# ZhangYizhao/UltraRE

Measured on AMD Instinct MI355X. Metric: training interactions/sec + unlearn retrain wall-time, ml-1m 5-shard SISA, higher is better.
Workload: dtype f32; 1 GPU; ml1m-shaped synthetic 6040x3416, 896914 train rows, 5-shard SISA (uniform grouping), d=32, batch=30000, SGD-momentum-L2, all shards of a rank side by side; parallelism=shards x1, arch=gfx950:sramecc+:xnack-

## Files before the change

include/ultrare_hip.h:

```cpp
#ifndef ULTRARE_HIP_H
#define ULTRARE_HIP_H

#include <stdint.h>

#ifdef __cplusplus
extern "C" {
#endif

#define URE_ABI_VERSION 15
#define URE_MAX_MODELS_PER_CALL 32
#define URE_SCORE_PARTIALS 2048

int ure_abi_version(void);
const char *ure_source_hash(void);
const char *ure_last_error(void);
int ure_device_info(int dev, int *n_cu, int *wave_size, char *arch, int arch_len);

typedef struct ure_shard {
    const int32_t *ent_oid;
    const float   *ent_r;
    uint16_t      *ent_tag;
    const int32_t *ent_src;
    uint16_t      *file_tag;
    uint32_t      *inv_stage;
// ... 32 lines not shown
typedef struct ure_job ure_job_t;

int ure_job_create(const ure_shard_t *shards, int n_shards, ure_job_t **out);

int ure_copy_rows_batch(int32_t n, const float *const *src, float *const *dst, float *const *dst2, const int64_t *rows, int32_t k, int32_t d,
                        void *stream);

int ure_epoch_sse_batch(int32_t n, const float *const *sse, const int64_t *n_user, int32_t epochs, double *out, void *stream);
int ure_job_destroy(ure_job_t *job);
int64_t ure_job_shard_steps(const ure_job_t *job, int s);
int64_t ure_job_ticks(const ure_job_t *job);

int ure_job_train(ure_job_t *job, int64_t tick0, int64_t tick1, void *stream);
int ure_job_materialize(ure_job_t *job, int64_t ticks_done, void *stream);
int ure_job_touch_rows(ure_job_t *job, int64_t *pairs, int64_t *window_steps);
int ure_job_index_read(ure_job_t *job, int shard, int which, void *out, int64_t capacity, int64_t *bytes);
int ure_job_train_profiled(ure_job_t *job, int64_t tick0, int64_t tick1, void *stream, double *step_ms,
                           int64_t *n_step, double *assign_ms, int64_t *n_assign);

int ure_host_randperm(const int64_t *seeds, int n_perms, int64_t n, int32_t *out, int n_threads);
int ure_host_randperm_tags(const int64_t *seeds, int n_perms, int64_t n, int32_t batch, uint16_t *tags, int n_threads);
typedef struct ure_perm {
    int64_t   seed;
    uint16_t *tags;
    int32_t   n;
    int32_t   batch;
} ure_perm_t;
int64_t ure_device_randperm_tags_scratch(int64_t n_max, int32_t groups);
int ure_device_randperm_tags(const ure_perm_t *perms, int32_t n_perms, int64_t n_max, uint32_t *scratch, int64_t scratch_words, int32_t groups,
                             void *stream);
// ... 147 lines not shown
```

ultrare_amd/_native.py:

```python
import ctypes
import os

import numpy as np

_PKG = os.path.dirname(os.path.abspath(__file__))
LIB_PATH = os.path.join(_PKG, 'libultrare_hip.so')
ABI_VERSION = 15
MAX_MODELS_PER_CALL = 32

_vp = ctypes.c_void_p
_i32 = ctypes.c_int32
_i64 = ctypes.c_int64


class UreShard(ctypes.Structure):
    _fields_ = [
        ('ent_oid', _vp), ('ent_r', _vp), ('ent_tag', _vp), ('ent_src', _vp), ('file_tag', _vp), ('inv_stage', _vp), ('inv_off', _vp),
        ('sched', _vp), ('units', _vp), ('n_units', _i32), ('n_active', _i32), ('n_slots', _i64),
        ('U', _vp * 2), ('V', _vp * 2), ('mU', _vp), ('mV', _vp),
        ('U0', _vp), ('V0', _vp), ('lr_host', _vp), ('lazy_rows', _i32),
        ('snapU', _vp), ('snapV', _vp), ('snap_a', _vp), ('snap', _vp), ('row_slot', _vp),
        ('perm', _vp), ('lr', _vp), ('sse', _vp),
        ('N', _i32), ('n_user', _i32), ('n_item', _i32), ('d', _i32),
        ('batch', _i32), ('epochs', _i32),
# ... 10 lines not shown
_PROTOTYPES = {
    'ure_abi_version': (ctypes.c_int, []),
    'ure_source_hash': (ctypes.c_char_p, []),
    'ure_last_error': (ctypes.c_char_p, []),
    'ure_device_info': (ctypes.c_int, [ctypes.c_int, ctypes.POINTER(ctypes.c_int), ctypes.POINTER(ctypes.c_int),
                                       ctypes.c_char_p, ctypes.c_int]),
    'ure_job_create': (ctypes.c_int, [ctypes.POINTER(UreShard), ctypes.c_int, ctypes.POINTER(_vp)]),
    'ure_job_destroy': (ctypes.c_int, [_vp]),
    'ure_copy_rows_batch': (ctypes.c_int, [_i32, _vp, _vp, _vp, _vp, _i32, _i32, _vp]),
    'ure_epoch_sse_batch': (ctypes.c_int, [_i32, _vp, _vp, _i32, _vp, _vp]),
    'ure_job_shard_steps': (_i64, [_vp, ctypes.c_int]),
    'ure_job_ticks': (_i64, [_vp]),
    'ure_job_train': (ctypes.c_int, [_vp, _i64, _i64, _vp]),
    'ure_job_materialize': (ctypes.c_int, [_vp, _i64, _vp]),
    'ure_job_touch_rows': (ctypes.c_int, [_vp, _vp, _vp]),
    'ure_job_index_read': (ctypes.c_int, [_vp, ctypes.c_int, ctypes.c_int, _vp, _i64, ctypes.POINTER(_i64)]),
    'ure_job_train_profiled': (ctypes.c_int, [_vp, _i64, _i64, _vp, ctypes.POINTER(ctypes.c_double), ctypes.POINTER(_i64),
                                              ctypes.POINTER(ctypes.c_double), ctypes.POINTER(_i64)]),
    'ure_host_randperm': (ctypes.c_int, [_vp, ctypes.c_int, _i64, _vp, ctypes.c_int]),
    'ure_host_randperm_tags': (ctypes.c_int, [_vp, ctypes.c_int, _i64, _i32, _vp, ctypes.c_int]),
    'ure_device_randperm_tags_scratch': (_i64, [_i64, _i32]),
    'ure_device_randperm_tags': (ctypes.c_int, [_vp, _i32, _i64, _vp, _i64, _i32, _vp]),
    'ure_device_shuffle_tags_scratch': (_i64, [_i64, _i32]),
    'ure_device_shuffle_tags_flag': (_i64, [_i64, _i32]),
    'ure_device_shuffle_tags': (ctypes.c_int, [_vp, _i32, _i64, _vp, _i64, _i32, _vp]),
    'ure_host_mt_advance': (ctypes.c_int, [_vp, _i64, _i64]),
    'ure_host_mt_jump_blocks': (ctypes.c_int, [_vp, _i64]),
    'ure_host_mt_jump_support': (ctypes.c_int, [_i64, _vp, _i32, ctypes.POINTER(_i32)]),
    'ure_host_mt_charpoly': (ctypes.c_int, [_vp, _i32]),
    'ure_host_draw_int64': (ctypes.c_int, [_vp, _i64, _i64, _i64, _vp]),
# ... 319 lines not shown
```

ultrare_amd/build.py:

```python
import os
import shutil
import subprocess
import sys

PKG = os.path.dirname(os.path.abspath(__file__))
ROOT = os.path.dirname(PKG)
CSRC = os.path.join(PKG, 'csrc')
LIB = os.path.join(PKG, 'libultrare_hip.so')
SOURCES = ['ure_common.hip', 'block_cache.cpp', 'mf_train.hip', 'tag_prep.hip', 'mf_eval.hip', 'mf_combine.hip', 'mf_ridge.hip', 'mf_recommend.hip', 'mf_rank.hip', 'pair_dist.hip', 'job_io.hip', 'perm_tags.hip', 'perm_chain.hip', 'mf_init.hip', 'ot.hip', 'ot_sinkhorn.hip', 'csr_group.hip', 'ot_solver.cpp', 'host_rng.cpp', 'mt_jump.cpp', 'host_layout.cpp']
FLAGS = ['-O3', '--offload-arch=gfx950', '-std=c++17', '-fPIC', '-shared', '-munsafe-fp-atomics',
         '-ffp-contract=off', '-Wall', '-Wno-unused-result', '-pthread', '-mllvm', '-amdgpu-kernarg-preload-count=8']


AVX2_SOURCE = 'host_normal_avx2.cpp'
AVX2_FLAGS = ['-O3', '-std=c++17', '-fPIC', '-mavx2', '-mfma', '-ffp-contract=fast', '-c']


def torch_include():
    try:
        import importlib.util
        spec = importlib.util.find_spec('torch')
        inc = os.path.join(os.path.dirname(spec.origin), 'include')
        return inc if os.path.exists(os.path.join(inc, 'ATen', 'native', 'cpu', 'avx_mathfun.h')) else None
    except Exception:
        return None


def source_hash(extra=()):
    import hashlib
    h = hashlib.sha256()
    files = sorted(os.path.join(CSRC, f) for f in os.listdir(CSRC) if not f.startswith('.')) + [os.path.join(ROOT, 'include', 'ultrare_hip.h')]
    for path in files:
        h.update(os.path.basename(path).encode() + b'\0')
        with open(path, 'rb') as f:
            h.update(f.read())
    h.update(' '.join(list(FLAGS) + list(extra) + AVX2_FLAGS + [str(torch_include() is not None)]).encode())
    return h.hexdigest()[:16]


STEP_KERNEL_FILES = ['mf_train.hip', 'mf_job.h', 'mf_touch.h', 'mf_index.h', 'tag_prep.h', 'tag_prep.hip', 'ure_internal.h']


def step_kernel_hash():
    import hashlib
    h = hashlib.sha256()
    for path in [os.path.join(CSRC, f) for f in STEP_KERNEL_FILES]:
        h.update(os.path.basename(path).encode() + b'\0')
        with open(path, 'rb') as f:
            h.update(f.read())
    with open(os.path.join(ROOT, 'include', 'ultrare_hip.h')) as f:
        text = f.read()
    a, b = text.index('typedef struct ure_shard'), text.index('} ure_shard_t;')
    h.update(text[a:b].encode())
    h.update(' '.join(FLAGS).encode())
    return h.hexdigest()[:16]
# ... 47 lines not shown
```

ultrare_amd/csrc/mf_job.h:

```cpp
#pragma once
#include <memory>

namespace ure {


static int check_descriptor(const ure_shard_t *shards, int k)
{
    const ure_shard_t &S = shards[k];
    const int n_rows = S.n_user + S.n_item;
    const bool ok = S.N > 0 && S.n_user > 0 && S.n_item > 0 && S.batch > 0 && S.epochs > 0 && pow2(S.d) && S.d >= 4 &&
                    S.d <= 256 && S.n_active >= 0 && S.n_active <= n_rows && S.units && S.n_units >= 0 &&
                    S.n_units % (kBlock / lanes_per_row(S.d)) == 0 && S.n_slots >= S.N && S.ent_oid && S.ent_r && S.ent_tag && S.ent_src &&
                    S.file_tag && S.sched && S.U[0] && S.U[1] && S.V[0] && S.V[1] && S.mU && S.mV && (S.perm || S.file_tags) && S.lr && S.sse &&
                    (!S.lazy_rows || (S.U0 && S.V0 && S.lr_host));
    if (!ok) return fail(-1, "ure_job_create: shard %d has an invalid descriptor", k);
    if (S.d != shards[0].d) return fail(-1, "ure_job_create: all shards of a job share d");
    const int steps = make_shard_aux(S).steps;
    if (steps > 65534) return fail(-1, "ure_job_create: shard %d needs %lld steps/epoch (> 65534)", k, (long long)steps);
    if (S.touch_mode && (S.n_multi < 0 || S.n_multi > S.n_active)) return fail(-1, "ure_job_create: shard %d: n_multi outside [0, n_active]", k);
    if (tag_partitioned(S.N) && !(S.inv_stage && S.inv_off)) return fail(-1, "ure_job_create: shard %d lacks inv_stage / inv_off", k);
    return 0;
}

static bool snapshot_set_ok(const ure_shard_t &S)
// ... 29 lines not shown
    }
    for (int k = 0; k < n_shards; ++k)
        if (!snapshot_set_ok(shards[k])) return fail(-1, "ure_job_create: shard %d has an incomplete snapshot set (full: snapU + snapV; compact: snap with lazy_rows; snap_a with lazy_rows)", k);
    for (int k = 0; k < n_shards && touch; ++k)
        if (const char *why = touch_refusal(shards, k, make_shard_aux(shards[k]).steps)) return fail(-1, "ure_job_create: touch mode refused for shard %d: %s", k, why);
    return 0;
}


static void plan_job(ure_job *job, const ure_shard_t *shards, int n_shards)
{
    job->host.assign(shards, shards + n_shards);
    job->d = shards[0].d;
    if (const char *e = std::getenv("URE_SHARD_FAST")) { job->shard_fast = e[0] != '0'; job->shard_sliced = e[0] == '2'; }
    if (const char *e = std::getenv("URE_INDEX_STAGED")) job->scatter_staged = e[0] != '0';
    job->ahead = shards[0].touch_mode == 2;
    job->index = shards[0].touch_mode == 3;
    for (int k = 0; k < n_shards; ++k) {
        const ure_shard_t &S = shards[k];
        const shard_aux A = make_shard_aux(S);
        const int n_rows = S.n_user + S.n_item, per_block = kBlock / lanes_per_row(S.d);
        job->aux_host.push_back(A);
        job->lr_host.emplace_back(S.lr_host ? std::vector<float>(S.lr_host, S.lr_host + S.epochs) : std::vector<float>());
        job->host[k].lr_host = nullptr;
        job->ticks = std::max(job->ticks, (int64_t)A.steps * S.epochs);
        job->row_blocks.push_back(S.touch_mode ? S.n_units / per_block + (S.n_active - S.n_multi + kBlock - 1) / kBlock
                                               : S.n_units / per_block + (S.lazy_rows ? 0 : (n_rows - S.n_active + per_block - 1) / per_block));
        job->max_n = std::max(job->max_n, S.N);
        job->max_slots = std::max(job->max_slots, S.n_slots);
        const bool small = tag_partitioned(S.N);
// ... 132 lines not shown
    int tab_n = kTouchTab;
    if (job->index)
        for (const shard_aux &A : job->aux_host) tab_n = std::max(tab_n, A.steps + 1);
    for (shard_aux &A : job->aux_host) A.ptab_stride = tab_n;
    const std::vector<float> tab = closed_form_table(job, tab_n);
    float4 *ptab = nullptr;
    if (hipError_t e = job_block(job, tab.size() * sizeof(float), kNoFill, &ptab)) return e;
    if (hipError_t e = hipMemcpy(ptab, tab.data(), tab.size() * sizeof(float), hipMemcpyHostToDevice)) return e;
    bool index_short = true;
    for (const shard_aux &A : job->aux_host) index_short = index_short && A.steps <= kIdxWin;
    for (int k = 0; k < (int)job->host.size(); ++k)
        if (hipError_t e = job->index ? index_memory(job, k, ptab, index_short) : window_memory(job, k, ptab)) return e;
    return hipSuccess;
}

static hipError_t upload_job(ure_job *job)
{
    const size_t n = job->host.size();
    if (hipError_t e = hipMalloc(&job->dev, sizeof(ure_shard_t) * n)) return e;
    if (hipError_t e = hipMemcpy(job->dev, job->host.data(), sizeof(ure_shard_t) * n, hipMemcpyHostToDevice)) return e;
    if (hipError_t e = hipMalloc(&job->dev_ab, sizeof(double) * 2 * n)) return e;
    if (job->touch)
        if (hipError_t e = touch_memory(job)) return e;
    if (hipError_t e = hipMalloc(&job->dev_aux, sizeof(shard_aux) * n)) return e;
    return hipMemcpy(job->dev_aux, job->aux_host.data(), sizeof(shard_aux) * n, hipMemcpyHostToDevice);
}

}

extern "C" int ure_job_create(const ure_shard_t *shards, int n_shards, ure_job_t **out)
{
    URE_ARG(shards && out && n_shards > 0 && n_shards <= 65535);
    if (int rc = ure::check_shards(shards, n_shards)) return rc;
    auto *job = new ure::ure_job();
    std::unique_ptr<ure_job_t, decltype(&ure_job_destroy)> hold(reinterpret_cast<ure_job_t *>(job), ure_job_destroy);
    ure::plan_job(job, shards, n_shards);
    const hipError_t e = ure::upload_job(job);
    if (e != hipSuccess) return ure::fail((int)e, "ure_job_create: %s", hipGetErrorString(e));
// ... 16 lines not shown
```

ultrare_amd/csrc/mf_train.hip:

```cpp
#include "tag_prep.h"

#include <algorithm>
#include <cstdlib>
#include <type_traits>
#include <vector>

#ifndef URE_KGB_NARROW
#define URE_KGB_NARROW 5
#endif
#ifndef URE_KGB_D16
#define URE_KGB_D16 5
#endif
#ifndef URE_WAVES_D16
#define URE_WAVES_D16 5
#endif
#ifndef URE_KGB_D8
#define URE_KGB_D8 5
#endif
#ifndef URE_WAVES_D8
#define URE_WAVES_D8 5
#endif
#ifndef URE_KGB_WIDE
#define URE_KGB_WIDE 4
#endif
// ... 35 lines not shown

template <int LPR, int V4>
__device__ __forceinline__ void mf_step(const ure_shard_t *__restrict__ shards, const shard_aux *__restrict__ aux, int64_t tick, int shard_fast)
{
    constexpr int D = LPR * V4 * 4;
    using Row = RowVec<V4>;
    constexpr int G = kWave / LPR;
    constexpr int UPB = kBlock / LPR;
    constexpr int CAP = kSegPerLane * LPR;
    constexpr int kGB = step_kgb(LPR, V4);
    constexpr int kQueueBytes = kWavesPerBlock * kQueue * 8;
    static_assert(kTagLds <= kQueueBytes, "tag phases must fit in the queue space");
    __shared__ __attribute__((aligned(16))) char lds_raw[kQueueBytes];
    __shared__ float4 part_acc[UPB][V4][LPR];
    int (*q_oid)[kQueue] = reinterpret_cast<int (*)[kQueue]>(lds_raw);
    float (*q_r)[kQueue] = reinterpret_cast<float (*)[kQueue]>(lds_raw + kWavesPerBlock * kQueue * 4);

    int shard_idx = (int)(shard_fast ? blockIdx.x : blockIdx.y);
    int wg = (int)(shard_fast ? blockIdx.y : blockIdx.x);
    if (shard_fast >> 1) {
        const unsigned n_sh = (unsigned)shard_fast >> 8;
        const unsigned x = blockIdx.x & 7u, j = blockIdx.x >> 3;
        const unsigned jq = j / n_sh, jr = j - jq * n_sh;
        const unsigned slice = n_sh * x + jr;
        shard_idx = (int)(slice >> 3);
        wg = (int)(jq * 8 + (slice & 7u));
    }
    const ure_shard_t &S = shards[shard_idx];
    const shard_aux &A = aux[shard_idx];
    {
        const int p_epochs = S.epochs, p_nu = S.n_user, p_ni = S.n_item, p_units = S.n_units, p_act = S.n_active, p_lazy = S.lazy_rows;
        const int64_t p_slots = S.n_slots;
        const float p_lam = S.lam, p_mu = S.mu;
        asm volatile("" ::"s"(p_epochs), "s"(p_nu), "s"(p_ni), "s"(p_units), "s"(p_act), "s"(p_lazy), "s"(p_slots), "s"(p_lam), "s"(p_mu),
                     "s"(S.lr), "s"(S.sched), "s"(S.units), "s"(S.ent_oid), "s"(S.ent_r), "s"(S.ent_tag), "s"(S.U[0]), "s"(S.U[1]),
                     "s"(S.V[0]), "s"(S.V[1]), "s"(S.mU), "s"(S.mV), "s"(S.sse), "s"(A.steps), "s"(A.inv_steps), "s"(A.ride_m),
                     "s"(A.ride_ab), "s"(A.ride_c), "s"(A.ranges), "s"(A.derive_blocks));
    }
    const int steps = A.steps;
    if (tick >= (int64_t)steps * S.epochs) return;
    const int epoch = (int)epoch_of(A, tick);
    const int s = (int)(tick - (int64_t)epoch * steps);
    const int cur = (int)(tick & 1);
    const bool first = tick == 0;
    const int n_rows = S.n_user + S.n_item;
    const int wave = threadIdx.x >> 6, lane = threadIdx.x & 63;
    const int sub = lane & (LPR - 1), grp = lane / LPR;
    const float lam = S.lam, mu = S.mu, lr = ldg(S.lr + epoch);
    const int32_t *__restrict__ ent_oid = S.ent_oid;
    const float *__restrict__ ent_r = S.ent_r;
    const uint16_t *__restrict__ ent_tag = S.ent_tag + (size_t)(epoch & 1) * S.n_slots;
    int *qo = q_oid[wave];
    float *qr = q_r[wave];

    auto sgd_update = [&](const Row &wr, const Row &mr, const Row &ar, float *mom_row, float *next_row, float *snap_row) {
        Row gr, nr;
#pragma unroll
        for (int i = 0; i < V4; ++i) {
            const float4 w = wr.q[i], m4 = mr.q[i], acc = ar.q[i];
            float4 g, wn;
            g.x = fmaf(lam, w.x, acc.x); g.y = fmaf(lam, w.y, acc.y);
            g.z = fmaf(lam, w.z, acc.z); g.w = fmaf(lam, w.w, acc.w);
            if (!first) {
                g.x = __fadd_rn(__fmul_rn(mu, m4.x), g.x); g.y = __fadd_rn(__fmul_rn(mu, m4.y), g.y);
                g.z = __fadd_rn(__fmul_rn(mu, m4.z), g.z); g.w = __fadd_rn(__fmul_rn(mu, m4.w), g.w);
            }
            wn.x = fmaf(-lr, g.x, w.x); wn.y = fmaf(-lr, g.y, w.y);
            wn.z = fmaf(-lr, g.z, w.z); wn.w = fmaf(-lr, g.w, w.w);
// ... 10 lines not shown
    const TagRide ride = tag_ride(A, s, epoch + 1 < S.epochs);
    const int nbR = ride.count;
    const int nbRows = nbU + nbD;
    const int blk = wg;
    if (blk >= nbRows) {
        const int rb = blk - nbRows;
        if (rb >= nbR) return;
        if (ride.phase == 0) tag_partition(S, epoch + 1, ride.first + rb, lds_raw);
        else if (ride.phase == 1) tag_collect(S, ride.first + rb, lds_raw);
        else tag_derive(S, epoch + 1, ride.first + rb, A.derive_blocks);
        return;
    }
    const int local = wave * G + grp;
    const bool dense_only = blk >= nbU;
    int4 du = make_int4(-1, 0, 0, local | (1 << 16));
    if (dense_only) {
        const int idx = S.n_active + (blk - nbU) * UPB + local;
        if (idx < n_rows) du.x = ldg(S.sched + 4 * (size_t)idx);
    } else {
        du = ldg_i4(S.units + 4 * ((size_t)blk * UPB + local));
    }
    const bool have = du.x >= 0;
    const int leader = du.w & 0xFFFF, count = (du.w >> 16) & 0x3FFF;
    const bool multi = (du.w >> 30) & 1;
    const bool owner = have && local == leader;
    const bool is_user = du.x < S.n_user;
    const int row = is_user ? du.x : du.x - S.n_user;
    const size_t row_off = (size_t)(have ? row : 0) * D;
    Row w = row_zero<V4>(), m4 = w, acc = w;
    if (have) {
        w = row_load<LPR, V4>((is_user ? S.U[cur] : S.V[cur]) + row_off, sub);
    }
    if (owner && !first) m4 = row_load<LPR, V4>((is_user ? S.mU : S.mV) + row_off, sub);
    const bool snap_here = S.snap != nullptr && S.row_slot != nullptr && s == steps - 1;
    int snap_slot = -1;
    if (snap_here && owner) snap_slot = ldg(S.row_slot + du.x);
    float sse = 0.f;
    URE_STAMP(2);
    if (!dense_only) {
        const float *__restrict__ other = is_user ? S.V[cur] : S.U[cur];
        int *gq = qo + grp * CAP;
        float *gr = qr + grp * CAP;
        const int beg = du.y, end = have ? du.z : 0;
        for (int seg = beg;; seg += CAP) {
            if (!__any(seg < end)) break;
            const int p0 = seg + sub * kSegPerLane;
            const bool valid = p0 < end;
            uint4 t4 = make_uint4(0xFFFFFFFFu, 0xFFFFFFFFu, 0xFFFFFFFFu, 0xFFFFFFFFu);
            int4 o0 = make_int4(0, 0, 0, 0), o1 = o0;
            float4 r0 = make_float4(0.f, 0.f, 0.f, 0.f), r1 = r0;
            if (valid) {
                t4 = ldg_u4(ent_tag + p0);
                o0 = ldg_i4(ent_oid + p0);
                o1 = ldg_i4(ent_oid + p0 + 4);
                r0 = ldg_f4(ent_r + p0);
                r1 = ldg_f4(ent_r + p0 + 4);
            }
            const unsigned tw[4] = {t4.x, t4.y, t4.z, t4.w};
            const int ov[8] = {o0.x, o0.y, o0.z, o0.w, o1.x, o1.y, o1.z, o1.w};
            const float rv[8] = {r0.x, r0.y, r0.z, r0.w, r1.x, r1.y, r1.z, r1.w};
            unsigned mb = 0;
#pragma unroll
            for (int k = 0; k < 8; ++k) {
                const unsigned tg = (tw[k >> 1] >> ((k & 1) * 16)) & 0xFFFFu;
                mb |= (tg == (unsigned)s ? 1u : 0u) << k;
            }
            const int c = __popc(mb);
            const int inc = group_scan<LPR>(c, sub);
            const int qn = (int)group_sum<LPR>((float)c);
            int mpos = inc - c, upos = qn + sub * kSegPerLane - mpos;
#pragma unroll
            for (int k = 0; k < 8; ++k) {
                const bool hit = (mb >> k) & 1u;
                const int pos = ((hit ? mpos : upos) + grp) & (CAP - 1);
                gq[pos] = ov[k];
                gr[pos] = rv[k];
                mpos += hit ? 1 : 0;
                upos += hit ? 0 : 1;
            }
            __builtin_amdgcn_wave_barrier();
            if (seg == beg) URE_STAMP(3);
            for (int t0 = 0; __any(t0 < qn); t0 += kGB) {
                int o[kGB];
                float r[kGB];
                bool act[kGB];
                Row v[kGB];
#pragma unroll
                for (int k = 0; k < kGB; ++k) {
                    const int qi = (min(t0 + k, CAP - 1) + grp) & (CAP - 1);
                    act[k] = t0 + k < qn;
                    o[k] = gq[qi];
                    r[k] = gr[qi];
                }
#pragma unroll
                for (int k = 0; k < kGB; ++k) v[k] = row_load<LPR, V4>(other + (size_t)(act[k] ? o[k] : 0) * D, sub);
#pragma unroll
                for (int k = 0; k < kGB; ++k) {
                    const float p = group_sum<LPR>(row_dot<V4>(w, v[k]));
                    const float e = p - r[k];
                    const float ge = act[k] ? 2.0f * e : 0.0f;
                    if (act[k]) sse = fmaf(e, e, sse);
                    row_axpy<V4>(acc, ge, v[k]);
                }
            }
            __builtin_amdgcn_wave_barrier();
        }
        URE_STAMP(4);
        if (multi) {
            if (have && count > 1) {
#pragma unroll
                for (int i = 0; i < V4; ++i) part_acc[local][i][sub] = acc.q[i];
                if (sub == 0) qr[grp * CAP] = sse;
            }
            __syncthreads();
            if (owner && count > 1) {
#pragma unroll
                for (int i = 0; i < V4; ++i) {
                    float4 a4 = part_acc[leader][i][sub];
                    for (int k = 1; k < count; ++k) {
                        const float4 t = part_acc[leader + k][i][sub];
                        a4.x += t.x; a4.y += t.y; a4.z += t.z; a4.w += t.w;
                    }
                    acc.q[i] = a4;
                }
                sse = 0.f;
                for (int k = 0; k < count; ++k) sse += q_r[(leader + k) / G][((leader + k) % G) * CAP];
            }
        }
    }
    if (owner) {
        sgd_update(w, m4, acc, (is_user ? S.mU : S.mV) + row_off, (is_user ? S.U[cur ^ 1] : S.V[cur ^ 1]) + row_off,
                   snap_slot >= 0 ? S.snap + ((size_t)epoch * S.n_active + snap_slot) * D : nullptr);
        if (is_user && sub == 0 && sse != 0.f) {
            float *slot = S.sse + (size_t)epoch * S.n_user + row;
            stg(slot, ldg(slot) + sse);
        }
    }
}

template <int LPR, int V4>
__global__ __launch_bounds__(kBlock) __attribute__((amdgpu_waves_per_eu(step_waves(LPR, V4)))) void mf_step_kernel(const ure_shard_t *__restrict__ shards, const shard_aux *__restrict__ aux, int64_t tick, int shard_fast)
// ... 353 lines not shown
    auto mark = [&](std::vector<hipEvent_t> *v) -> int {
        if (!v) return 0;
        hipEvent_t e;
        URE_HIP(hipEventCreate(&e));
        v->push_back(e);
        URE_HIP(hipEventRecord(e, st));
        return 0;
    };
    auto timed = [&](std::vector<hipEvent_t> *v, auto launches) -> int {
        if (int rc = mark(v)) return rc;
        if (!launches()) return fail(-1, "ure_job_train: unsupported d=%d", job->d);
        return mark(v);
    };
    for (int64_t t = tick0; t < tick1; ++t) {
        int rc = 0;
        if (const int passes = tag_prep_needed(job, t))
            rc = timed(assign_ev, [&] {
                if (passes & 1) launch_tag_prep(job, t, st, 0);
                if (passes & 2) launch_tag_prep(job, t, st, 1);
                return true;
            });
        if (rc) return rc;
        if (job->ahead && touch_prep_needed(job, t))
            rc = timed(assign_ev, [&] { return with_width(job->d, [&](auto lpr, auto v4) { launch_touch_ahead<decltype(lpr)::value, decltype(v4)::value>(job, t, st); }); });
        else if (index_epoch_start_needed(job, t))
            rc = timed(assign_ev, [&] { launch_index_epoch_start(job, t, st); return true; });
        else if (touch_prep_needed(job, t))
            rc = timed(assign_ev, [&] { return with_width(job->d, [&](auto lpr, auto) { launch_touch_prep<decltype(lpr)::value>(job, t, st); }); });
        if (rc) return rc;
        rc = timed(step_ev, [&] { return with_width(job->d, [&](auto lpr, auto v4) { launch_step<decltype(lpr)::value, decltype(v4)::value>(job, t, st); }); });
// ... 76 lines not shown
        const ure_shard_t &S = job->host[k];
        const shard_aux &A = job->aux_host[k];
        const int64_t steps = A.steps;
        const int64_t last = std::min<int64_t>(job->next_tick, steps * S.epochs) - 1;
        const int64_t epoch = last / steps, win = (last % steps) / kTouchWindow;
        host.resize((size_t)S.n_user + S.n_item);
        URE_HIP(hipMemcpy(host.data(), A.mask[(epoch * A.windows + win) & 1], host.size() * sizeof(unsigned long long), hipMemcpyDeviceToHost));
        int64_t n = 0;
        for (unsigned long long m : host) n += __builtin_popcountll(job->ahead ? m & ~(1ull << 63) : m);
        pairs[k] = n;
        window_steps[k] = std::min<int64_t>(kTouchWindow, steps - win * kTouchWindow);
    }
    return 0;
}

int ure_job_index_read(ure_job_t *j, int shard, int which, void *out, int64_t capacity, int64_t *bytes)
{
    auto *job = reinterpret_cast<ure::ure_job *>(j);
    URE_ARG(job && shard >= 0 && shard < (int)job->host.size() && bytes);
    if (!job->index) return fail(-1, "ure_job_index_read: the job is not in touch_mode 3");
    const ure_shard_t &S = job->host[(size_t)shard];
    const shard_aux &A = job->aux_host[(size_t)shard];
    URE_HIP(hipDeviceSynchronize());
    uint32_t n_items = 0, total = 0;
    URE_HIP(hipMemcpy(&n_items, A.step_item + A.steps, 4, hipMemcpyDeviceToHost));
    URE_HIP(hipMemcpy(&total, A.step_begin + A.steps, 4, hipMemcpyDeviceToHost));
    const void *src = nullptr;
    size_t n = 0;
    switch (which) {
        case 0: src = A.step_begin; n = ((size_t)A.steps + 1) * 4; break;
// ... 58 lines not shown
```

ultrare_amd/csrc/tag_prep.h:

```cpp
#pragma once
#include "ure_internal.h"

namespace ure {

constexpr int kRange = 2048;
constexpr int kMaxRanges = 1024;
constexpr int kRangeBits = 11;
static_assert((1 << kRangeBits) == kRange, "range size");

__host__ __device__ inline int tag_ranges(int n) { return (n + kRange - 1) / kRange; }
__host__ __device__ inline bool tag_partitioned(int n) { return tag_ranges(n) <= kMaxRanges; }

constexpr int kTagLdsA = (kMaxRanges + 1) * 4 + kRange * 4 + kBlock * 4;
constexpr int kTagLdsB = kRange * 2 + 2 * kMaxRanges * 4;
constexpr int kTagLds = kTagLdsA > kTagLdsB ? kTagLdsA : kTagLdsB;

struct BatchOf {
    unsigned long long M;
    __device__ explicit BatchOf(int batch) : M((0x4000000000000000ull + (unsigned long long)batch - 1) / (unsigned long long)batch) {}
    __device__ __forceinline__ int operator()(int b) const { return (int)__umul64hi((unsigned long long)b << 2, M); }
};

__device__ inline void tag_partition(const ure_shard_t &S, int epoch, int c, char *lds)
{
// ... 158 lines not shown
    uint32_t *hist;
    uint32_t *seg;
    uint32_t *step_begin;
    uint4 *sslot;
    unsigned long long *runflag;
    uint32_t *blk_cnt;
    int4 *items;
    uint4 *items2;
    uint32_t *step_item;
    uint32_t *heavy_cnt;
    uint32_t *heavy_cum;
    uint32_t *heavy_map;
    uint32_t *heavy_wg;
    uint4 *step_desc;
    float *partial;
};

constexpr int kTouchWindow = 64;
constexpr int kTouchWindowBits = 6;
__host__ __device__ inline int64_t touch_last_window(const shard_aux &a, int64_t epoch) { return (epoch + 1) * a.windows - 1; }

__host__ __device__ inline bool tag_short_riders(const ure_shard_t &S)
{
    const int64_t steps = ((int64_t)S.N + S.batch - 1) / S.batch;
    return steps < 3 && S.file_tags != nullptr && S.touch_mode != 3;
}
__host__ __device__ inline bool tag_riders(const ure_shard_t &S)
{
    const int64_t steps = ((int64_t)S.N + S.batch - 1) / S.batch;
    return ((steps >= 3 && tag_partitioned(S.N)) || tag_short_riders(S)) && S.touch_mode != 3;
// ... 58 lines not shown
```

ultrare_amd/csrc/ure_internal.h:

```cpp
#pragma once
#include <hip/hip_runtime.h>

#include <algorithm>
#include <cstdarg>
#include <cstdint>
#include <cstdio>
#include <vector>

#include "ultrare_hip.h"

#ifndef URE_NARROW_MAX
#define URE_NARROW_MAX 32
#endif

namespace ure {

constexpr int kWave = 64;
constexpr int kBlock = 256;
constexpr int kWavesPerBlock = kBlock / kWave;

char *err_buf();
int fail(int code, const char *fmt, ...);
int host_threads();

// ... 25 lines not shown
    std::vector<std::vector<float>> lr_host;
    std::vector<double> ab_host;
    double *dev_ab = nullptr;
    std::vector<struct shard_aux> aux_host;
    struct shard_aux *dev_aux = nullptr;
    bool shard_sliced = true;
    bool shard_fast = true;
    bool snapshots = false;
    unsigned snap_blocks = 1;
    int64_t max_lazy = 0;
    bool touch = false;
    bool ahead = false;
    bool index = false;
    bool index_split = false;
    bool scatter_staged = true;
    bool all_file_tags = true;
    std::vector<void *> touch_mem;
    int max_units = 0;
    int64_t max_active4 = 0;
    int max_rows = 0;
};

int tag_prep_needed(const ure_job *job, int64_t tick);
void launch_tag_prep(const ure_job *job, int64_t tick, hipStream_t st, int pass);

hipError_t block_malloc(void **out, size_t bytes);
void block_free(void *p);

#define URE_AS1 __attribute__((address_space(1)))
typedef float ure_f4 __attribute__((ext_vector_type(4)));
// ... 134 lines not shown
```

ultrare_amd/engine.py:

```python
import contextlib
import ctypes
import math
import os

import numpy as np
import torch

from . import _native as nv

SCORE_PARTIALS = 2048
SERIES_SCRATCH_BYTES = 256 << 20
LAZY_ROWS = os.environ.get('URE_LAZY_ROWS', '1') != '0'
TOUCH_MAX_STEPS = 32000
TOUCH_ROW_PASSES = 2
TOUCH_UNIT_PASSES = 8
TOUCH_AHEAD_MAX_STEPS = 63
INDEX_MAX_STEPS = 1008
INDEX_HEAVY_SLOTS = 16
INDEX_SPLIT_SLOTS = 384
INDEX_HEAVY_MAX = 256
INDEX_SHORT_EPOCH_MAX_D = 64
TOUCH_MIN_TABLE_BYTES = 256 << 20


# ... 574 lines not shown
        return U[:, :self.k], V[:, :self.k]

    def padded_tables(self, s):
        self.materialize()
        cur = min(self.done, self.shard_steps[s]) & 1
        st = self.state[s]
        return st['U'][cur], st['V'][cur]

    def touch_rows_per_step(self):
        if not self.touch:
            return None
        out, win = np.zeros(len(self.shards), dtype=np.int64), np.zeros(len(self.shards), dtype=np.int64)
        nv.check(nv.lib().ure_job_touch_rows(self._job, out.ctypes.data, win.ctypes.data), 'ure_job_touch_rows')
        return [float(n) / max(int(w), 1) for n, w in zip(out, win)]

    _INDEX_ARRAYS = {'step_begin': (0, np.uint32, 1), 'step_item': (1, np.uint32, 1), 'items': (2, np.int32, 4), 'sslot': (3, np.uint32, 4),
                     'W': (4, np.uint64, 1), 'heavy_cnt': (5, np.uint32, 1), 'heavy_cum': (6, np.uint32, 257)}

    def index_array(self, s, name):
        which, dtype, cols = self._INDEX_ARRAYS[name]
        n = ctypes.c_int64()
        nv.check(nv.lib().ure_job_index_read(self._job, s, which, None, 0, ctypes.byref(n)), 'ure_job_index_read')
        out = np.empty(n.value // np.dtype(dtype).itemsize, dtype=dtype)
        nv.check(nv.lib().ure_job_index_read(self._job, s, which, out.ctypes.data, out.nbytes, ctypes.byref(n)), 'ure_job_index_read')
        return out.reshape(-1, cols) if cols > 1 else out

    def epoch_sse(self, s):
        return self.epoch_sse_queue([s]).cpu().numpy()[0]

    def epoch_sse_queue(self, which=None, out=None, stream=None):
# ... 735 lines not shown
```

Before: 7.681 billion interactions/s.

## Pack slot ids to 16-bit and ratings to 8-bit dictionary codes

Adds a one-time preprocessing pass at tick 0 that builds a per-shard dictionary of distinct rating values (up to 256). When ids fit in 16 bits, it re-encodes entity ids as uint16 and ratings as uint8 codes. The training scan then reads the packed arrays and looks up ratings in the dictionary, which cuts streamed bytes per slot from 8 to 3. The cost is extra pack kernels on the first tick and a dictionary gather per interaction. Shards with too many distinct ratings or too many ids fall back to the unpacked path.

```diff
diff --git a/include/ultrare_hip.h b/include/ultrare_hip.h
--- a/include/ultrare_hip.h
+++ b/include/ultrare_hip.h
@@ -70,6 +70,7 @@
 int ure_job_train(ure_job_t *job, int64_t tick0, int64_t tick1, void *stream);
 int ure_job_materialize(ure_job_t *job, int64_t ticks_done, void *stream);
 int ure_job_touch_rows(ure_job_t *job, int64_t *pairs, int64_t *window_steps);
+int ure_job_slots_packed(ure_job_t *job, int shard);
 int ure_job_index_read(ure_job_t *job, int shard, int which, void *out, int64_t capacity, int64_t *bytes);
 int ure_job_train_profiled(ure_job_t *job, int64_t tick0, int64_t tick1, void *stream, double *step_ms,
                            int64_t *n_step, double *assign_ms, int64_t *n_assign);
diff --git a/ultrare_amd/_native.py b/ultrare_amd/_native.py
--- a/ultrare_amd/_native.py
+++ b/ultrare_amd/_native.py
@@ -48,6 +48,7 @@
     'ure_job_train': (ctypes.c_int, [_vp, _i64, _i64, _vp]),
     'ure_job_materialize': (ctypes.c_int, [_vp, _i64, _vp]),
     'ure_job_touch_rows': (ctypes.c_int, [_vp, _vp, _vp]),
+    'ure_job_slots_packed': (ctypes.c_int, [_vp, ctypes.c_int]),
     'ure_job_index_read': (ctypes.c_int, [_vp, ctypes.c_int, ctypes.c_int, _vp, _i64, ctypes.POINTER(_i64)]),
     'ure_job_train_profiled': (ctypes.c_int, [_vp, _i64, _i64, _vp, ctypes.POINTER(ctypes.c_double), ctypes.POINTER(_i64),
                                               ctypes.POINTER(ctypes.c_double), ctypes.POINTER(_i64)]),
diff --git a/ultrare_amd/build.py b/ultrare_amd/build.py
--- a/ultrare_amd/build.py
+++ b/ultrare_amd/build.py
@@ -38,7 +38,7 @@
     return h.hexdigest()[:16]
 
 
-STEP_KERNEL_FILES = ['mf_train.hip', 'mf_job.h', 'mf_touch.h', 'mf_index.h', 'tag_prep.h', 'tag_prep.hip', 'ure_internal.h']
+STEP_KERNEL_FILES = ['mf_train.hip', 'mf_job.h', 'mf_touch.h', 'mf_index.h', 'slot_pack.h', 'tag_prep.h', 'tag_prep.hip', 'ure_internal.h']
 
 
 def step_kernel_hash():
diff --git a/ultrare_amd/csrc/mf_job.h b/ultrare_amd/csrc/mf_job.h
--- a/ultrare_amd/csrc/mf_job.h
+++ b/ultrare_amd/csrc/mf_job.h
@@ -67,6 +67,7 @@
     job->d = shards[0].d;
     if (const char *e = std::getenv("URE_SHARD_FAST")) { job->shard_fast = e[0] != '0'; job->shard_sliced = e[0] == '2'; }
     if (const char *e = std::getenv("URE_INDEX_STAGED")) job->scatter_staged = e[0] != '0';
+    if (const char *e = std::getenv("URE_SLOT_PACK")) job->slot_pack = e[0] != '0';
     job->ahead = shards[0].touch_mode == 2;
     job->index = shards[0].touch_mode == 3;
     for (int k = 0; k < n_shards; ++k) {
@@ -229,6 +230,33 @@
     return hipSuccess;
 }
 
+static size_t carve_pack(ure_job *job, void *base)
+{
+    Carve c{reinterpret_cast<uintptr_t>(base)};
+    uint32_t *flags = nullptr;
+    c.take(flags, job->host.size() * sizeof(uint32_t));
+    for (size_t k = 0; k < job->host.size(); ++k) {
+        const ure_shard_t &S = job->host[k];
+        shard_aux &A = job->aux_host[k];
+        A.pk_flag = flags + k;
+        if (!job->slot_pack || S.n_user > kPackIdMax || S.n_item > kPackIdMax) continue;
+        c.take(A.pk_oid, (size_t)S.n_slots * sizeof(uint16_t));
+        c.take(A.pk_r, (size_t)S.n_slots);
+        c.take(A.r_dict, kPackDict * sizeof(float));
+        c.take(A.pk_set, kPackSet * sizeof(unsigned long long));
+        c.take(A.pk_count, sizeof(uint32_t));
+    }
+    return c.at;
+}
+
+static hipError_t pack_memory(ure_job *job)
+{
+    char *mem = nullptr;
+    if (hipError_t e = job_block(job, carve_pack(job, nullptr), kNoFill, &mem)) return e;
+    carve_pack(job, mem);
+    return hipSuccess;
+}
+
 static hipError_t upload_job(ure_job *job)
 {
     const size_t n = job->host.size();
@@ -237,6 +265,8 @@
     if (hipError_t e = hipMalloc(&job->dev_ab, sizeof(double) * 2 * n)) return e;
     if (job->touch)
         if (hipError_t e = touch_memory(job)) return e;
+    if (!job->touch)
+        if (hipError_t e = pack_memory(job)) return e;
     if (hipError_t e = hipMalloc(&job->dev_aux, sizeof(shard_aux) * n)) return e;
     return hipMemcpy(job->dev_aux, job->aux_host.data(), sizeof(shard_aux) * n, hipMemcpyHostToDevice);
 }
diff --git a/ultrare_amd/csrc/mf_train.hip b/ultrare_amd/csrc/mf_train.hip
--- a/ultrare_amd/csrc/mf_train.hip
+++ b/ultrare_amd/csrc/mf_train.hip
@@ -1,4 +1,5 @@
 #include "tag_prep.h"
+#include "slot_pack.h"
 
 #include <algorithm>
 #include <cstdlib>
@@ -73,7 +74,7 @@
     __shared__ __attribute__((aligned(16))) char lds_raw[kQueueBytes];
     __shared__ float4 part_acc[UPB][V4][LPR];
     int (*q_oid)[kQueue] = reinterpret_cast<int (*)[kQueue]>(lds_raw);
-    float (*q_r)[kQueue] = reinterpret_cast<float (*)[kQueue]>(lds_raw + kWavesPerBlock * kQueue * 4);
+    unsigned (*q_r)[kQueue] = reinterpret_cast<unsigned (*)[kQueue]>(lds_raw + kWavesPerBlock * kQueue * 4);
 
     int shard_idx = (int)(shard_fast ? blockIdx.x : blockIdx.y);
     int wg = (int)(shard_fast ? blockIdx.y : blockIdx.x);
@@ -94,7 +95,7 @@
         asm volatile("" ::"s"(p_epochs), "s"(p_nu), "s"(p_ni), "s"(p_units), "s"(p_act), "s"(p_lazy), "s"(p_slots), "s"(p_lam), "s"(p_mu),
                      "s"(S.lr), "s"(S.sched), "s"(S.units), "s"(S.ent_oid), "s"(S.ent_r), "s"(S.ent_tag), "s"(S.U[0]), "s"(S.U[1]),
                      "s"(S.V[0]), "s"(S.V[1]), "s"(S.mU), "s"(S.mV), "s"(S.sse), "s"(A.steps), "s"(A.inv_steps), "s"(A.ride_m),
-                     "s"(A.ride_ab), "s"(A.ride_c), "s"(A.ranges), "s"(A.derive_blocks));
+                     "s"(A.ride_ab), "s"(A.ride_c), "s"(A.ranges), "s"(A.derive_blocks), "s"(A.pk_oid), "s"(A.pk_r), "s"(A.r_dict), "s"(A.pk_flag));
     }
     const int steps = A.steps;
     if (tick >= (int64_t)steps * S.epochs) return;
@@ -109,8 +110,11 @@
     const int32_t *__restrict__ ent_oid = S.ent_oid;
     const float *__restrict__ ent_r = S.ent_r;
     const uint16_t *__restrict__ ent_tag = S.ent_tag + (size_t)(epoch & 1) * S.n_slots;
+    const uint16_t *__restrict__ pk_oid = A.pk_oid;
+    const uint8_t *__restrict__ pk_r = A.pk_r;
+    const float URE_AS1 *__restrict__ r_dict = (const float URE_AS1 *)A.r_dict;
     int *qo = q_oid[wave];
-    float *qr = q_r[wave];
+    unsigned *qr = q_r[wave];
 
     auto sgd_update = [&](const Row &wr, const Row &mr, const Row &ar, float *mom_row, float *next_row, float *snap_row) {
         Row gr, nr;
@@ -151,6 +155,7 @@
     const int local = wave * G + grp;
     const bool dense_only = blk >= nbU;
     int4 du = make_int4(-1, 0, 0, local | (1 << 16));
+    const bool packed = ldg(A.pk_flag) != 0u;
     if (dense_only) {
         const int idx = S.n_active + (blk - nbU) * UPB + local;
         if (idx < n_rows) du.x = ldg(S.sched + 4 * (size_t)idx);
@@ -177,77 +182,113 @@
     if (!dense_only) {
         const float *__restrict__ other = is_user ? S.V[cur] : S.U[cur];
         int *gq = qo + grp * CAP;
-        float *gr = qr + grp * CAP;
+        unsigned *gr = qr + grp * CAP;
         const int beg = du.y, end = have ? du.z : 0;
-        for (int seg = beg;; seg += CAP) {
-            if (!__any(seg < end)) break;
-            const int p0 = seg + sub * kSegPerLane;
-            const bool valid = p0 < end;
-            uint4 t4 = make_uint4(0xFFFFFFFFu, 0xFFFFFFFFu, 0xFFFFFFFFu, 0xFFFFFFFFu);
-            int4 o0 = make_int4(0, 0, 0, 0), o1 = o0;
-            float4 r0 = make_float4(0.f, 0.f, 0.f, 0.f), r1 = r0;
-            if (valid) {
-                t4 = ldg_u4(ent_tag + p0);
-                o0 = ldg_i4(ent_oid + p0);
-                o1 = ldg_i4(ent_oid + p0 + 4);
-                r0 = ldg_f4(ent_r + p0);
-                r1 = ldg_f4(ent_r + p0 + 4);
+        auto scan_units = [&](auto packed_t) {
+            constexpr bool kPacked = decltype(packed_t)::value;
+            for (int seg = beg;; seg += CAP) {
+                if (!__any(seg < end)) break;
+                const int p0 = seg + sub * kSegPerLane;
+                const bool valid = p0 < end;
+                uint4 t4 = make_uint4(0xFFFFFFFFu, 0xFFFFFFFFu, 0xFFFFFFFFu, 0xFFFFFFFFu);
+                int ov[8];
+                unsigned rv[8];
+                if (kPacked) {
+                    uint4 o = make_uint4(0u, 0u, 0u, 0u);
+                    ure_u2 c;
+                    c.x = c.y = 0u;
+                    if (valid) {
+                        t4 = ldg_u4(ent_tag + p0);
+                        o = ldg_u4(pk_oid + p0);
+                        c = *(const ure_u2 URE_AS1 *)(pk_r + p0);
+                    }
+                    const unsigned ow[4] = {o.x, o.y, o.z, o.w};
+    #pragma unroll
+                    for (int k = 0; k < 8; ++k) {
+                        ov[k] = (int)((ow[k >> 1] >> ((k & 1) * 16)) & 0xFFFFu);
+                        rv[k] = ((k < 4 ? c.x : c.y) >> ((k & 3) * 8)) & 0xFFu;
+                    }
+                } else {
+                    int4 o0 = make_int4(0, 0, 0, 0), o1 = o0;
+                    uint4 r0 = make_uint4(0u, 0u, 0u, 0u), r1 = r0;
+                    if (valid) {
+                        t4 = ldg_u4(ent_tag + p0);
+                        o0 = ldg_i4(ent_oid + p0);
+                        o1 = ldg_i4(ent_oid + p0 + 4);
+                        r0 = ldg_u4(ent_r + p0);
+                        r1 = ldg_u4(ent_r + p0 + 4);
+                    }
+                    ov[0] = o0.x; ov[1] = o0.y; ov[2] = o0.z; ov[3] = o0.w; ov[4] = o1.x; ov[5] = o1.y; ov[6] = o1.z; ov[7] = o1.w;
+                    rv[0] = r0.x; rv[1] = r0.y; rv[2] = r0.z; rv[3] = r0.w; rv[4] = r1.x; rv[5] = r1.y; rv[6] = r1.z; rv[7] = r1.w;
+                }
+                const unsigned tw[4] = {t4.x, t4.y, t4.z, t4.w};
+                unsigned mb = 0;
+    #pragma unroll
+                for (int k = 0; k < 8; ++k) {
+                    const unsigned tg = (tw[k >> 1] >> ((k & 1) * 16)) & 0xFFFFu;
+                    mb |= (tg == (unsigned)s ? 1u : 0u) << k;
+                }
+                const int c = __popc(mb);
+                const int inc = group_scan<LPR>(c, sub);
+                const int qn = (int)group_sum<LPR>((float)c);
+                int mpos = inc - c, upos = qn + sub * kSegPerLane - mpos;
+    #pragma unroll
+                for (int k = 0; k < 8; ++k) {
+                    const bool hit = (mb >> k) & 1u;
+                    const int pos = ((hit ? mpos : upos) + grp) & (CAP - 1);
+                    gq[pos] = ov[k];
+                    gr[pos] = rv[k];
+                    mpos += hit ? 1 : 0;
+                    upos += hit ? 0 : 1;
+                }
+                __builtin_amdgcn_wave_barrier();
+                if (seg == beg) URE_STAMP(3);
+                for (int t0 = 0; __any(t0 < qn); t0 += kGB) {
+                    int o[kGB];
+                    unsigned rb[kGB];
+                    float r[kGB];
+                    bool act[kGB];
+                    Row v[kGB];
+    #pragma unroll
+                    for (int k = 0; k < kGB; ++k) {
+                        const int qi = (min(t0 + k, CAP - 1) + grp) & (CAP - 1);
+                        act[k] = t0 + k < qn;
+                        o[k] = gq[qi];
+                        rb[k] = gr[qi];
+                    }
+                    if (kPacked) {
+    #pragma unroll
+                        for (int k = 0; k < kGB; ++k) {
+                            r[k] = r_dict[rb[k] & (unsigned)(kPackDict - 1)];
+                            v[k] = row_load<LPR, V4>(other + (size_t)(act[k] ? o[k] : 0) * D, sub);
+                        }
+                    } else {
+    #pragma unroll
+                        for (int k = 0; k < kGB; ++k) {
+                            r[k] = __uint_as_float(rb[k]);
+                            v[k] = row_load<LPR, V4>(other + (size_t)(act[k] ? o[k] : 0) * D, sub);
+                        }
+                    }
+    #pragma unroll
+                    for (int k = 0; k < kGB; ++k) {
+                        const float p = group_sum<LPR>(row_dot<V4>(w, v[k]));
+                        const float e = p - r[k];
+                        const float ge = act[k] ? 2.0f * e : 0.0f;
+                        if (act[k]) sse = fmaf(e, e, sse);
+                        row_axpy<V4>(acc, ge, v[k]);
+                    }
+                }
+                __builtin_amdgcn_wave_barrier();
             }
-            const unsigned tw[4] = {t4.x, t4.y, t4.z, t4.w};
-            const int ov[8] = {o0.x, o0.y, o0.z, o0.w, o1.x, o1.y, o1.z, o1.w};
-            const float rv[8] = {r0.x, r0.y, r0.z, r0.w, r1.x, r1.y, r1.z, r1.w};
-            unsigned mb = 0;
-#pragma unroll
-            for (int k = 0; k < 8; ++k) {
-                const unsigned tg = (tw[k >> 1] >> ((k & 1) * 16)) & 0xFFFFu;
-                mb |= (tg == (unsigned)s ? 1u : 0u) << k;
-            }
-            const int c = __popc(mb);
-            const int inc = group_scan<LPR>(c, sub);
-            const int qn = (int)group_sum<LPR>((float)c);
-            int mpos = inc - c, upos = qn + sub * kSegPerLane - mpos;
-#pragma unroll
-            for (int k = 0; k < 8; ++k) {
-                const bool hit = (mb >> k) & 1u;
-                const int pos = ((hit ? mpos : upos) + grp) & (CAP - 1);
-                gq[pos] = ov[k];
-                gr[pos] = rv[k];
-                mpos += hit ? 1 : 0;
-                upos += hit ? 0 : 1;
-            }
-            __builtin_amdgcn_wave_barrier();
-            if (seg == beg) URE_STAMP(3);
-            for (int t0 = 0; __any(t0 < qn); t0 += kGB) {
-                int o[kGB];
-                float r[kGB];
-                bool act[kGB];
-                Row v[kGB];
-#pragma unroll
-                for (int k = 0; k < kGB; ++k) {
-                    const int qi = (min(t0 + k, CAP - 1) + grp) & (CAP - 1);
-                    act[k] = t0 + k < qn;
-                    o[k] = gq[qi];
-                    r[k] = gr[qi];
-                }
-#pragma unroll
-                for (int k = 0; k < kGB; ++k) v[k] = row_load<LPR, V4>(other + (size_t)(act[k] ? o[k] : 0) * D, sub);
-#pragma unroll
-                for (int k = 0; k < kGB; ++k) {
-                    const float p = group_sum<LPR>(row_dot<V4>(w, v[k]));
-                    const float e = p - r[k];
-                    const float ge = act[k] ? 2.0f * e : 0.0f;
-                    if (act[k]) sse = fmaf(e, e, sse);
-                    row_axpy<V4>(acc, ge, v[k]);
-                }
-            }
-            __builtin_amdgcn_wave_barrier();
-        }
+        };
+        if (packed) scan_units(std::true_type{});
+        else scan_units(std::false_type{});
         URE_STAMP(4);
         if (multi) {
             if (have && count > 1) {
 #pragma unroll
                 for (int i = 0; i < V4; ++i) part_acc[local][i][sub] = acc.q[i];
-                if (sub == 0) qr[grp * CAP] = sse;
+                if (sub == 0) qr[grp * CAP] = __float_as_uint(sse);
             }
             __syncthreads();
             if (owner && count > 1) {
@@ -261,7 +302,7 @@
                     acc.q[i] = a4;
                 }
                 sse = 0.f;
-                for (int k = 0; k < count; ++k) sse += q_r[(leader + k) / G][((leader + k) % G) * CAP];
+                for (int k = 0; k < count; ++k) sse += __uint_as_float(q_r[(leader + k) / G][((leader + k) % G) * CAP]);
             }
         }
     }
@@ -645,6 +686,7 @@
     };
     for (int64_t t = tick0; t < tick1; ++t) {
         int rc = 0;
+        if (t == 0 && !job->touch) URE_HIP(launch_slot_pack(job, st));
         if (const int passes = tag_prep_needed(job, t))
             rc = timed(assign_ev, [&] {
                 if (passes & 1) launch_tag_prep(job, t, st, 0);
@@ -751,6 +793,17 @@
     return 0;
 }
 
+int ure_job_slots_packed(ure_job_t *j, int shard)
+{
+    auto *job = reinterpret_cast<ure::ure_job *>(j);
+    if (!job || shard < 0 || shard >= (int)job->host.size()) return ure::fail(-1, "ure_job_slots_packed: no such shard");
+    if (job->touch || job->next_tick == 0) return 0;
+    uint32_t flag = 0;
+    if (hipDeviceSynchronize() != hipSuccess || hipMemcpy(&flag, job->aux_host[(size_t)shard].pk_flag, sizeof(flag), hipMemcpyDeviceToHost) != hipSuccess)
+        return ure::fail(-1, "ure_job_slots_packed: the flag of shard %d could not be read", shard);
+    return flag != 0;
+}
+
 int ure_job_index_read(ure_job_t *j, int shard, int which, void *out, int64_t capacity, int64_t *bytes)
 {
     auto *job = reinterpret_cast<ure::ure_job *>(j);
diff --git a/ultrare_amd/csrc/slot_pack.h b/ultrare_amd/csrc/slot_pack.h
--- /dev/null
+++ b/ultrare_amd/csrc/slot_pack.h
@@ -0,0 +1,180 @@
+#pragma once
+#include "tag_prep.h"
+
+namespace ure {
+
+constexpr int kPackDict = 256;
+constexpr int kPackIdMax = 65536;
+constexpr int kPackSet = 1024;
+constexpr unsigned kPackOverflow = 0x80000000u;
+constexpr unsigned long long kPackTaken = 1ull << 32;
+
+__device__ __forceinline__ unsigned pack_hash(unsigned bits) { return (bits * 2654435761u) >> 22; }
+static_assert(kPackSet == 1 << 10, "pack_hash yields 10 bits");
+
+__global__ __launch_bounds__(kBlock) void slot_pack_clear_kernel(const shard_aux *__restrict__ aux)
+{
+    const shard_aux &A = aux[blockIdx.x];
+    if (threadIdx.x == 0) stg(A.pk_flag, 0u);
+    if (!A.pk_set) return;
+    for (int t = threadIdx.x; t < kPackSet; t += kBlock) stg(A.pk_set + t, 0ull);
+    if (threadIdx.x == 0) stg(A.pk_count, 0u);
+}
+
+__global__ __launch_bounds__(kBlock) void slot_pack_collect_kernel(const ure_shard_t *__restrict__ shards, const shard_aux *__restrict__ aux)
+{
+    __shared__ unsigned long long set[kPackSet];
+    __shared__ unsigned n_set;
+    const ure_shard_t &S = shards[blockIdx.y];
+    const shard_aux &A = aux[blockIdx.y];
+    if (!A.pk_set) return;
+    const int64_t n8 = S.n_slots / 8;
+    if ((int64_t)blockIdx.x * kBlock >= n8) return;
+    for (int t = threadIdx.x; t < kPackSet; t += kBlock) set[t] = 0ull;
+    if (threadIdx.x == 0) n_set = 0;
+    __syncthreads();
+    const float *__restrict__ ent_r = S.ent_r;
+    const int32_t *__restrict__ ent_src = S.ent_src;
+    unsigned last = 0;
+    bool have_last = false;
+    for (int64_t q = (int64_t)blockIdx.x * kBlock + threadIdx.x; q < n8; q += (int64_t)gridDim.x * kBlock) {
+        const uint4 a = ldg_u4(ent_r + q * 8), b = ldg_u4(ent_r + q * 8 + 4);
+        const int4 s0 = ldg_i4(ent_src + q * 8), s1 = ldg_i4(ent_src + q * 8 + 4);
+        const unsigned v[8] = {a.x, a.y, a.z, a.w, b.x, b.y, b.z, b.w};
+        const int src[8] = {s0.x, s0.y, s0.z, s0.w, s1.x, s1.y, s1.z, s1.w};
+#pragma unroll
+        for (int k = 0; k < 8; ++k) {
+            if (src[k] < 0 || (have_last && v[k] == last)) continue;
+            last = v[k];
+            have_last = true;
+            const unsigned long long key = kPackTaken | v[k];
+            unsigned h = pack_hash(v[k]);
+            int probe = 0;
+            for (; probe < kPackSet; ++probe, h = (h + 1) & (kPackSet - 1)) {
+                unsigned long long cur = *(volatile unsigned long long *)&set[h];
+                if (cur == key) break;
+                if (cur != 0ull) continue;
+                if (*(volatile unsigned *)&n_set > (unsigned)kPackDict) break;
+                cur = atomicCAS(&set[h], 0ull, key);
+                if (cur == 0ull) { atomicAdd(&n_set, 1u); break; }
+                if (cur == key) break;
+            }
+            if (probe == kPackSet) atomicAdd(&n_set, (unsigned)kPackDict + 1u);
+        }
+    }
+    __syncthreads();
+    if (n_set > (unsigned)kPackDict) {
+        if (threadIdx.x == 0) __hip_atomic_fetch_or(A.pk_count, kPackOverflow, __ATOMIC_RELAXED, __HIP_MEMORY_SCOPE_AGENT);
+        return;
+    }
+    for (int t = threadIdx.x; t < kPackSet; t += kBlock) {
+        const unsigned long long key = set[t];
+        if (key == 0ull) continue;
+        unsigned h = pack_hash((unsigned)key);
+        int probe = 0;
+        for (; probe < kPackSet; ++probe, h = (h + 1) & (kPackSet - 1)) {
+            unsigned long long cur = __hip_atomic_load(A.pk_set + h, __ATOMIC_RELAXED, __HIP_MEMORY_SCOPE_AGENT);
+            if (cur == key) break;
+            if (cur != 0ull) continue;
+            if (__hip_atomic_load(A.pk_count, __ATOMIC_RELAXED, __HIP_MEMORY_SCOPE_AGENT) > (unsigned)kPackDict) break;
+            unsigned long long expect = 0ull;
+            if (__hip_atomic_compare_exchange_strong(A.pk_set + h, &expect, key, __ATOMIC_RELAXED, __ATOMIC_RELAXED, __HIP_MEMORY_SCOPE_AGENT)) {
+                __hip_atomic_fetch_add(A.pk_count, 1u, __ATOMIC_RELAXED, __HIP_MEMORY_SCOPE_AGENT);
+                break;
+            }
+            if (expect == key) break;
+        }
+        if (probe == kPackSet) __hip_atomic_fetch_or(A.pk_count, kPackOverflow, __ATOMIC_RELAXED, __HIP_MEMORY_SCOPE_AGENT);
+    }
+}
+
+__global__ __launch_bounds__(kBlock) void slot_pack_dict_kernel(const ure_shard_t *__restrict__ shards, const shard_aux *__restrict__ aux)
+{
+    __shared__ unsigned val[kPackDict];
+    __shared__ unsigned n_val;
+    const ure_shard_t &S = shards[blockIdx.x];
+    const shard_aux &A = aux[blockIdx.x];
+    if (!A.pk_set) return;
+    const unsigned count = ldg(A.pk_count);
+    if (count > (unsigned)kPackDict || S.n_user > kPackIdMax || S.n_item > kPackIdMax) return;
+    if (threadIdx.x == 0) n_val = 0;
+    __syncthreads();
+    for (int t = threadIdx.x; t < kPackSet; t += kBlock) {
+        const unsigned long long key = ldg(A.pk_set + t);
+        if (key == 0ull) continue;
+        const unsigned at = atomicAdd(&n_val, 1u);
+        if (at < (unsigned)kPackDict) val[at] = (unsigned)key;
+    }
+    __syncthreads();
+    const int t = threadIdx.x;
+    static_assert(kPackDict <= kBlock, "one thread per dictionary entry");
+    if (t < kPackDict) {
+        if (t < (int)n_val) {
+            const unsigned mine = val[t];
+            int rank = 0;
+            for (int k = 0; k < (int)n_val; ++k) rank += val[k] < mine ? 1 : 0;
+            stg(reinterpret_cast<unsigned *>(A.r_dict) + rank, mine);
+        } else {
+            stg(reinterpret_cast<unsigned *>(A.r_dict) + t, 0u);
+        }
+    }
+    if (t == 0) {
+        stg(A.pk_count, n_val);
+        stg(A.pk_flag, 1u);
+    }
+}
+
+__global__ __launch_bounds__(kBlock) void slot_pack_encode_kernel(const ure_shard_t *__restrict__ shards, const shard_aux *__restrict__ aux)
+{
+    __shared__ unsigned dict[kPackDict];
+    const ure_shard_t &S = shards[blockIdx.y];
+    const shard_aux &A = aux[blockIdx.y];
+    if (!A.pk_set || ldg(A.pk_flag) == 0u) return;
+    const int64_t n8 = S.n_slots / 8;
+    if ((int64_t)blockIdx.x * kBlock >= n8) return;
+    const unsigned n_val = ldg(A.pk_count);
+    if (threadIdx.x < kPackDict) dict[threadIdx.x] = threadIdx.x < n_val ? ldg(reinterpret_cast<const unsigned *>(A.r_dict) + threadIdx.x) : 0xFFFFFFFFu;
+    __syncthreads();
+    const int32_t *__restrict__ ent_oid = S.ent_oid;
+    const float *__restrict__ ent_r = S.ent_r;
+    for (int64_t q = (int64_t)blockIdx.x * kBlock + threadIdx.x; q < n8; q += (int64_t)gridDim.x * kBlock) {
+        const uint4 o0 = ldg_u4(ent_oid + q * 8), o1 = ldg_u4(ent_oid + q * 8 + 4);
+        const uint4 r0 = ldg_u4(ent_r + q * 8), r1 = ldg_u4(ent_r + q * 8 + 4);
+        const unsigned ov[8] = {o0.x, o0.y, o0.z, o0.w, o1.x, o1.y, o1.z, o1.w};
+        const unsigned rv[8] = {r0.x, r0.y, r0.z, r0.w, r1.x, r1.y, r1.z, r1.w};
+        unsigned code[8];
+#pragma unroll
+        for (int k = 0; k < 8; ++k) {
+            unsigned lo = 0;
+#pragma unroll
+            for (int step = kPackDict / 2; step >= 1; step >>= 1)
+                if (dict[lo + step - 1] < rv[k]) lo += step;
+            code[k] = lo;
+        }
+        stg_u4(A.pk_oid + q * 8, make_uint4((ov[0] & 0xFFFFu) | (ov[1] << 16), (ov[2] & 0xFFFFu) | (ov[3] << 16), (ov[4] & 0xFFFFu) | (ov[5] << 16),
+                                            (ov[6] & 0xFFFFu) | (ov[7] << 16)));
+        ure_u2 c;
+        c.x = code[0] | (code[1] << 8) | (code[2] << 16) | (code[3] << 24);
+        c.y = code[4] | (code[5] << 8) | (code[6] << 16) | (code[7] << 24);
+        *(ure_u2 URE_AS1 *)(A.pk_r + q * 8) = c;
+    }
+}
+
+static hipError_t launch_slot_pack(const ure_job *job, hipStream_t st)
+{
+    const unsigned n_sh = (unsigned)job->host.size();
+    hipLaunchKernelGGL(slot_pack_clear_kernel, dim3(n_sh), dim3(kBlock), 0, st, job->dev_aux);
+    if (hipError_t e = hipGetLastError()) return e;
+    if (!job->slot_pack) return hipSuccess;
+    const int64_t groups = (job->max_slots / 8 + kBlock - 1) / kBlock;
+    hipLaunchKernelGGL(slot_pack_collect_kernel, dim3((unsigned)std::max<int64_t>(1, std::min<int64_t>((groups + 3) / 4, 256)), n_sh), dim3(kBlock), 0, st,
+                       job->dev, job->dev_aux);
+    if (hipError_t e = hipGetLastError()) return e;
+    hipLaunchKernelGGL(slot_pack_dict_kernel, dim3(n_sh), dim3(kBlock), 0, st, job->dev, job->dev_aux);
+    if (hipError_t e = hipGetLastError()) return e;
+    hipLaunchKernelGGL(slot_pack_encode_kernel, dim3((unsigned)std::max<int64_t>(1, std::min<int64_t>(groups, 1024)), n_sh), dim3(kBlock), 0, st, job->dev,
+                       job->dev_aux);
+    return hipGetLastError();
+}
+
+}
diff --git a/ultrare_amd/csrc/tag_prep.h b/ultrare_amd/csrc/tag_prep.h
--- a/ultrare_amd/csrc/tag_prep.h
+++ b/ultrare_amd/csrc/tag_prep.h
@@ -196,6 +196,12 @@
     uint32_t *heavy_wg;
     uint4 *step_desc;
     float *partial;
+    uint32_t *pk_flag;
+    uint16_t *pk_oid;
+    uint8_t *pk_r;
+    float *r_dict;
+    unsigned long long *pk_set;
+    uint32_t *pk_count;
 };
 
 constexpr int kTouchWindow = 64;
diff --git a/ultrare_amd/csrc/ure_internal.h b/ultrare_amd/csrc/ure_internal.h
--- a/ultrare_amd/csrc/ure_internal.h
+++ b/ultrare_amd/csrc/ure_internal.h
@@ -63,6 +63,7 @@
     bool index = false;
     bool index_split = false;
     bool scatter_staged = true;
+    bool slot_pack = true;
     bool all_file_tags = true;
     std::vector<void *> touch_mem;
     int max_units = 0;
diff --git a/ultrare_amd/engine.py b/ultrare_amd/engine.py
--- a/ultrare_amd/engine.py
+++ b/ultrare_amd/engine.py
@@ -612,6 +612,11 @@
         nv.check(nv.lib().ure_job_touch_rows(self._job, out.ctypes.data, win.ctypes.data), 'ure_job_touch_rows')
         return [float(n) / max(int(w), 1) for n, w in zip(out, win)]
 
+    def slots_packed(self, s):
+        rc = int(nv.lib().ure_job_slots_packed(self._job, s))
+        nv.check(min(rc, 0), 'ure_job_slots_packed')
+        return rc == 1
+
     _INDEX_ARRAYS = {'step_begin': (0, np.uint32, 1), 'step_item': (1, np.uint32, 1), 'items': (2, np.int32, 4), 'sslot': (3, np.uint32, 4),
                      'W': (4, np.uint64, 1), 'heavy_cnt': (5, np.uint32, 1), 'heavy_cum': (6, np.uint32, 257)}
 
```

New measurement: 7.790 billion interactions/s, median of 6. 1.01x the previous value.
